# maxilevi/vits.cpp

Hardware: AMD Instinct MI355X
Metric: audio samples/sec end-to-end (ids -> fp32 PCM in HBM), vits-english architecture, batch=64 x 128 ids (higher is better)
Workload: dtype f32; 1 GPU; c3 b64x128 ref-mode f32 predicted-dur | vits-english = MMS-TTS arch, synthetic weights; batch_per_gpu=64, ids_per_utterance=128, parallelism=utterance-sharded x1

## Files before the change

### include/vits.h

```cpp
#ifndef VITS_HIP_H
#define VITS_HIP_H

#include <stddef.h>
#include <stdint.h>

#ifdef __cplusplus
#define VITS_API extern "C" __attribute__((visibility("default")))
#else
#define VITS_API __attribute__((visibility("default")))
#endif

typedef struct vits_model vits_model;

typedef struct vits_result {
    float* data;
    size_t size;
} vits_result;


VITS_API vits_model* vits_model_load_from_bytes(const char* bytes, size_t size);
VITS_API vits_model* vits_model_load_from_file(const char* path);
VITS_API void vits_free_model(vits_model* model);
VITS_API void vits_free_result(vits_result result);
VITS_API vits_result vits_model_process(vits_model* model, const char* phonemes);
// ... 204 lines not shown
    int32_t n, k[3], dilation;
    float slope;
} vits_conv_group_desc;
VITS_API int vits_op_conv_group(const vits_conv_group_desc* d, const float* x, const float* w, const float* bias, const int32_t* lens, float* y);

typedef struct vits_conv1d_desc {
    int32_t batch, cin, cout, t, t_stride;
    int32_t k, dilation, pad_left;
    int32_t pre_act;
    float pre_slope;
    int32_t post_act;
    float out_scale;
} vits_conv1d_desc;
VITS_API int vits_op_conv1d(const vits_conv1d_desc* d, const float* x, const float* w, const float* bias,
                            const float* residual, const float* accum, const int32_t* lens, float* y);

typedef struct vits_resblock_pair_desc {
    int32_t batch, channels, t, t_stride;
    int32_t k, dilation;
    float slope;
} vits_resblock_pair_desc;
VITS_API int vits_op_resblock_pair(const vits_resblock_pair_desc* d, const float* x, const float* w1, const float* b1,
                                   const float* w2, const float* b2, const int32_t* lens, float* y);

typedef struct vits_resblock_desc {
    int32_t batch, channels, t, t_stride;
    int32_t k, ndil;
    int32_t dil[3];
    float slope, out_scale;
    int32_t scale_div;
// ... 228 lines not shown
```

### vits.cpp_amd/__init__.py

```python
import ctypes as C
import json
import os

import numpy as np

_HERE = os.path.dirname(os.path.abspath(__file__))
LIB_PATH = os.environ.get("VITS_HIP_LIB", os.path.join(_HERE, "csrc", "libvits_hip.so"))

MODE_DEFAULT, MODE_REFERENCE, MODE_HF = -1, 0, 1
NOISE_REFERENCE, NOISE_COUNTER, NOISE_EXPLICIT = 0, 1, 2
SYNTH_FULL, SYNTH_TINY, SYNTH_BF16, SYNTH_SPEAKERS, SYNTH_POSTERIOR = 0, 1, 0x100, 0x200, 0x400
SYNTH_DETERMINISTIC = 0x800
DP_STOCHASTIC, DP_DETERMINISTIC = 0, 1
DP_VARIANT_PLAN, DP_VARIANT_LAT, DP_VARIANT_WIDE, DP_VARIANT_UNFUSED = 0, 1, 2, 3
RB_VARIANT_PLAN, RB_VARIANT_UNFUSED, RB_VARIANT_PAIRS, RB_VARIANT_BLOCK, RB_VARIANT_SEGMENTS = 0, 1, 2, 3, 4
FLOW_VARIANT_PLAN, FLOW_VARIANT_UNFUSED, FLOW_VARIANT_WAVENET, FLOW_VARIANT_COUPLING = 0, 1, 2, 3
UP16_VARIANT_PLAN, UP16_VARIANT_TILE, UP16_VARIANT_STREAM = 0, 1, 2
DDS_VARIANT_PLAN, DDS_VARIANT_UNFUSED, DDS_VARIANT_LAYER, DDS_VARIANT_LAT = 0, 1, 2, 3
DDS_HEAD_NONE, DDS_HEAD_FROM1, DDS_HEAD_CONV = 0, 1, 2
ATT_VARIANT_PLAN, ATT_VARIANT_VALU1024, ATT_VARIANT_VALU256, ATT_VARIANT_MFMA4, ATT_VARIANT_MFMA8, ATT_VARIANT_SHORT, ATT_VARIANT_LAT = 0, 1, 2, 3, 4, 5, 6
NC_VARIANT_PLAN, NC_VARIANT_SEPARATE, NC_VARIANT_ON_LOAD = 0, 1, 2
CONV_POST_FP32_LAYOUT, CONV_POST_STREAM = 0, 1
ARITH_F32, ARITH_BF16, ARITH_F16, ARITH_F32_SPLIT = 0, 1, 2, 3
LEVEL_NONE, LEVEL_MEASURE, LEVEL_GAIN, LEVEL_PEAK, LEVEL_LOUDNESS = 0, 1, 2, 3, 4
LIMIT_OFF, LIMIT_TRUE_PEAK = 0, 1
EDGES_OFF, EDGES_PAD, EDGES_TRIM_RELATIVE, EDGES_TRIM_ABSOLUTE = 0, 1, 2, 3
SCOPE_FLOW_VOCODER, SCOPE_ALL_CONVS = 0, 1

EXPORTED_SYMBOLS = [
    "vits_model_load_from_bytes", "vits_model_load_from_file", "vits_free_model", "vits_free_result",
    "vits_model_process", "vits_last_error", "vits_model_set_mode", "vits_model_get_mode",
    "vits_reference_noise_seed", "vits_model_process_ids", "vits_model_process_batch", "vits_free_batch_result",
    "vits_model_sync", "vits_model_tokenize", "vits_model_sampling_rate", "vits_model_vocab_size",
    "vits_model_weight_bytes", "vits_model_get_tap", "vits_synth_model_bytes", "vits_free_bytes",
    "vits_prof_enable", "vits_prof_reset", "vits_prof_report", "vits_op_conv1d", "vits_op_conv_transpose1d",
    "vits_op_rel_attention", "vits_op_add_layer_norm", "vits_device_info", "vits_set_device", "vits_model_file_reserialize",
    "vits_model_file_tokenize", "vits_pcm16_from_float", "vits_write_wav16", "vits_pcm16_from_float_device",
    "vits_model_set_arith", "vits_model_get_arith", "vits_model_file_validate", "vits_op_set_arith", "vits_op_tile_map_launches", "vits_op_set_output_fill", "vits_op_conv_group",
    "vits_model_set_arith_scope", "vits_model_get_arith_scope", "vits_model_submit_batch", "vits_model_wait", "vits_model_pending",
    "vits_model_set_ggml_tables", "vits_model_get_ggml_tables",
    "vits_model_set_speaker", "vits_model_get_speaker", "vits_model_num_speakers",
    "vits_model_speaker_embedding_size", "vits_model_get_speaker_embedding", "vits_model_add_voices", "vits_model_set_voice",
    "vits_model_clear_voices", "vits_model_num_voices",
    "vits_model_set_prosody", "vits_model_get_prosody",
    "vits_model_prepare_conversion", "vits_model_convert_batch", "vits_model_convert",
    "vits_model_align_batch", "vits_model_align", "vits_model_hop", "vits_op_align", "vits_op_resblock_pair",
    "vits_model_set_rates", "vits_model_get_rates", "vits_resample_plan", "vits_resample_taps", "vits_resample_length", "vits_op_resample",
    "vits_model_set_level", "vits_model_get_level", "vits_model_last_levels", "vits_loudness_plan", "vits_loudness_host", "vits_op_level",
    "vits_model_set_limiter", "vits_model_get_limiter", "vits_model_last_limits", "vits_limiter_plan", "vits_limiter_host", "vits_op_limit",
    "vits_model_set_edges", "vits_model_get_edges", "vits_model_last_edges", "vits_edges_plan", "vits_edges_host", "vits_op_edges",
    "vits_join_plan", "vits_join_host", "vits_op_join", "vits_split_sentences", "vits_model_process_joined", "vits_model_last_joins", "vits_model_speak",
    "vits_model_duration_predictor_kind", "vits_op_duration_predictor", "vits_op_resblock", "vits_op_resblock_plan",
    "vits_op_flow_coupling", "vits_op_flow_coupling_plan", "vits_op_upsample16", "vits_op_upsample16_plan",
# ... 45 lines not shown

class BatchResult(C.Structure):
    _fields_ = [("data", C.POINTER(C.c_float)), ("stride", C.c_size_t), ("lengths", C.POINTER(C.c_int64)),
                ("frames", C.POINTER(C.c_int64)), ("batch", C.c_size_t)]


class SpeakOpts(C.Structure):
    _fields_ = [("struct_size", C.c_uint32), ("sentence_gap_ms", C.c_float), ("paragraph_gap_ms", C.c_float), ("track_per_paragraph", C.c_int32),
                ("process", C.POINTER(ProcessOpts))]


class Conv1dDesc(C.Structure):
    _fields_ = [("batch", C.c_int32), ("cin", C.c_int32), ("cout", C.c_int32), ("t", C.c_int32), ("t_stride", C.c_int32),
                ("k", C.c_int32), ("dilation", C.c_int32), ("pad_left", C.c_int32), ("pre_act", C.c_int32),
                ("pre_slope", C.c_float), ("post_act", C.c_int32), ("out_scale", C.c_float)]


class ResblockPairDesc(C.Structure):
    _fields_ = [("batch", C.c_int32), ("channels", C.c_int32), ("t", C.c_int32), ("t_stride", C.c_int32), ("k", C.c_int32),
                ("dilation", C.c_int32), ("slope", C.c_float)]


class ConvGroupDesc(C.Structure):
    _fields_ = [("batch", C.c_int32), ("channels", C.c_int32), ("t", C.c_int32), ("t_stride", C.c_int32), ("n", C.c_int32), ("k", C.c_int32 * 3),
                ("dilation", C.c_int32), ("slope", C.c_float)]


class ResblockDesc(C.Structure):
    _fields_ = [("batch", C.c_int32), ("channels", C.c_int32), ("t", C.c_int32), ("t_stride", C.c_int32), ("k", C.c_int32), ("ndil", C.c_int32),
                ("dil", C.c_int32 * 3), ("slope", C.c_float), ("out_scale", C.c_float), ("scale_div", C.c_int32), ("variant", C.c_int32),
# ... 1059 lines not shown
              out_scale=1.0, lens=None):
    x, w = _f32(x), _f32(w)
    B, cin, T = x.shape
    cout, _, k = w.shape
    d = Conv1dDesc(B, cin, cout, T, T, k, dilation, (k - 1) * dilation // 2 if pad_left is None else pad_left,
                   0 if pre_slope is None else 1, 0.0 if pre_slope is None else pre_slope, post_act, out_scale)
    cy = cout // 2 if post_act == 2 else cout
    y = np.zeros((B, cy, T), np.float32)
    bias, residual, accum = _f32(bias), _f32(residual), _f32(accum)
    lens = None if lens is None else np.ascontiguousarray(lens, dtype=np.int32)
    if lib().vits_op_conv1d(C.byref(d), _ptr(x), _ptr(w), _ptr(bias), _ptr(residual), _ptr(accum), _ptr(lens), _ptr(y)) != 0:
        raise VitsError(last_error())
    return y


def op_resblock_pair(x, w1, b1, w2, b2, dilation, slope, lens=None):
    x, w1, w2, b1, b2 = _f32(x), _f32(w1), _f32(w2), _f32(b1), _f32(b2)
    B, ch, T = x.shape
    k = w1.shape[2]
    assert w1.shape == (ch, ch, k) and w2.shape == (ch, ch, k)
    d = ResblockPairDesc(B, ch, T, T, k, dilation, slope)
    y = np.zeros((B, ch, T), np.float32)
    lens = None if lens is None else np.ascontiguousarray(lens, dtype=np.int32)
    if lib().vits_op_resblock_pair(C.byref(d), _ptr(x), _ptr(w1), _ptr(b1), _ptr(w2), _ptr(b2), _ptr(lens), _ptr(y)) != 0:
        raise VitsError(last_error())
    return y


def _resblock_desc(B, ch, T, ts, k, dils, slope, out_scale, scale_div, variant, tiles, nr):
    dils = [int(v) for v in dils]
# ... 770 lines not shown
```

### vits.cpp_amd/csrc/abi_ops_common.h

```cpp
#pragma once
#include <algorithm>
#include <cstdint>
#include <cstring>
#include <memory>
#include <string>
#include <vector>

#include "../../include/vits.h"
#include "abi_internal.h"
#include "engine.h"

namespace vits {
extern thread_local int g_op_out_fill;
extern thread_local int g_op_arith;

inline bool refuse(const std::string& why) {
    set_err(why);
    return false;
}

struct DevMem {
    void* p = nullptr;
    DevMem() = default;
    DevMem(const DevMem&) = delete;
// ... 62 lines not shown
    for (int b = 0; b < batch; ++b)
        for (int c = 0; c < channels; ++c) {
            const T* g = &h[((size_t)b * channels + (size_t)(c / 8) * 8) * pitch + (c & 7)];
            T* d = dst + ((size_t)b * channels + c) * dst_pitch;
            for (int n = 0; n < t; ++n) d[n] = g[(size_t)n * 8];
        }
    return true;
}

struct OpKnobs {
    KernelKnobs k;
    KernelKnobsScope scope;
    OpKnobs() : k(kernel_knobs()), scope(&k) {
        k.no_tile_map = getenv("VITS_NO_TILE_MAP") != nullptr;
        k.tile_map = getenv("VITS_TILE_MAP") != nullptr;
    }
};
struct OpTileMaps {
    TileMapSet set;
    std::vector<std::unique_ptr<DevMem>> mem;
    bool add(const int32_t* len_in, const int32_t* len_out, int batch, int t_in, int t_out, int width, bool convt) {
        const KernelKnobs& kn = kernel_knobs();
        if (kn.no_tile_map || set.find(width, convt)) return true;
        std::vector<int> la(batch, t_in), lb(batch, t_out);
        if (len_in) la.assign(len_in, len_in + batch);
        if (len_out) lb.assign(len_out, len_out + batch);
        if (!kn.tile_map && !tile_map_needed(la.data(), lb.data(), batch, t_in, t_out, width, convt)) return true;
        std::vector<TileEntry> e((size_t)tile_map_count(la.data(), lb.data(), batch, width, convt) + 1);
        const int64_t n = tile_map_fill(la.data(), lb.data(), batch, width, convt, e.data());
        mem.emplace_back(new DevMem);
        if (!mem.back()->put(e.data(), e.size() * sizeof(TileEntry))) return false;
        return set.add(TileMapRef{static_cast<const TileEntry*>(mem.back()->p), (int)n, width, convt}) || refuse("too many tile widths for one length vector");
    }
    bool add_conv(const int32_t* len_in, const int32_t* len_out, int batch, int t_in, int t_out, bool convt) {
        return add(len_in, len_out, batch, t_in, t_out, tile_shape(TILE_128x128).bn(), convt) && add(len_in, len_out, batch, t_in, t_out, tile_shape(TILE_64x256).bn(), convt);
    }
};

struct Conv {
    PackedConv pc;
    DevMem w, wl, w16, b;
};
inline bool upload_conv(Conv& c, const float* w, const float* bias, size_t bias_n, int cout, int cin, int taps, int epi, int ct_stride, int arith, bool l16_always = false) {
    PackedConv& pc = c.pc;
    const ConvPackDims pd = conv_pack_dims(cout, cin, taps, epi, ct_stride);
    pc.cin = cin, pc.cout = cout, pc.kt = pd.kt, pc.epi = epi, pc.ct_stride = ct_stride;
    pc.rows = pd.rows, pc.mtiles_used = pd.mtiles_used, pc.mtiles = pd.mtiles, pc.nchunks = pd.nchunks;
    if (bias) {
        if (!c.b.put(bias, bias_n * 4)) return false;
        pc.bias = c.b.f();
// ... 34 lines not shown
```

### vits.cpp_amd/csrc/abi_ops_conv.cpp

```cpp
#include <cstdio>

#include "abi_ops_common.h"

namespace vits {
thread_local int g_op_arith = VITS_ARITH_F32;
thread_local int g_op_out_fill = 0;
}
using namespace vits;

namespace {
bool split3_nan(DevMem& d, int batch, int channels, int ts, Split3Ref* r) {
    if (!d.fill((size_t)batch * 3 * channels * ts * 2, 0xFF)) return false;
    r->p = d.h();
    r->ts = ts;
    r->ps = (int64_t)channels * ts;
    r->bs = 3 * r->ps;
    return true;
}
std::string split_refusal(int cin, int cout, int k, int dil) {
    char m[200] = "";
    if (cin < 128 || (cin & 31)) std::snprintf(m, sizeof(m), "VITS_ARITH_F32_SPLIT: c_in = %d is not taken by the split kernels (a multiple of 32, at least 128)", cin);
    else if (cout < 128 || (cout & 127)) std::snprintf(m, sizeof(m), "VITS_ARITH_F32_SPLIT: c_out = %d is not taken by the split kernels (a multiple of 128)", cout);
    else if (k != 3 && k != 7 && k != 11) std::snprintf(m, sizeof(m), "VITS_ARITH_F32_SPLIT: k = %d taps are not taken by the split kernels (3, 7 or 11)", k);
    else if (dil != 1 && dil != 3 && dil != 5) std::snprintf(m, sizeof(m), "VITS_ARITH_F32_SPLIT: dilation %d is not taken by the split kernels (1, 3 or 5)", dil);
// ... 97 lines not shown
        c.len_in = c.len_out = dl.i();
        c.maps = &maps.set;
        c.batch = B;
        c.t_in = c.t_out = d->t;
        c.dil = d->dilation;
        c.pad_l = (k * d->dilation - d->dilation) / 2;
        c.pre_act = 1, c.slope = d->slope, c.post_act = 2, c.post_slope = d->slope;
        pw[i] = &cv[i].pc;
    }
    return finish(launch_conv_group(pw, cc, n, nullptr), "vits_op_conv_group") && dy.get(y, per * n * 4) ? 0 : -1;
    VITS_CATCH(-1)
}

VITS_API uint64_t vits_op_tile_map_launches(void) { return tile_map_launches().load(std::memory_order_relaxed); }

VITS_API int vits_op_conv1d(const vits_conv1d_desc* d, const float* x, const float* w, const float* bias, const float* residual, const float* accum,
                            const int32_t* lens, float* y) {
    VITS_TRY
    if (!d || !x || !w || !y) return fail("null argument");
    const int arith = g_op_arith;
    if (arith == VITS_ARITH_F32_SPLIT) return op_conv1d_split(d, x, w, bias, residual, accum, lens, y);
    OpKnobs op_knobs;
    OpTileMaps maps;
    const int gate = d->post_act == 2;
    const int cy = gate ? d->cout / 2 : d->cout;
    Conv cv;
    DevMem dx, dy, dr, da, dl, x16;
    const size_t nx = (size_t)d->batch * d->cin * d->t_stride * 4, ny = (size_t)d->batch * cy * d->t_stride * 4;
    if (!upload_conv(cv, w, bias, d->cout, d->cout, d->cin, d->k, gate ? EPI_GATE : EPI_STD, 0, arith)) return -1;
    if (!dx.put(x, nx) || !dy.fill(ny, g_op_out_fill) || !dl.put_opt(lens, (size_t)d->batch * 4)) return -1;
    if ((residual && !dr.put(residual, ny)) || (accum && !da.put(accum, ny))) return -1;
    if (arith != VITS_ARITH_F32 && !x16.fill(group16_bytes(d->batch, d->cin, d->t), 0)) return -1;
    ConvCall c;
    c.x = tref(dx.f(), d->cin, d->t_stride);
    c.y = tref(dy.f(), cy, d->t_stride);
    if (residual) c.res = tref(dr.f(), cy, d->t_stride);
    if (accum) c.acc = tref(da.f(), cy, d->t_stride);
    c.len_in = dl.i();
    c.len_out = dl.i();
    c.batch = d->batch;
    c.t_in = c.t_out = d->t;
    c.dil = d->dilation;
    c.pad_l = d->pad_left;
    c.pre_act = d->pre_act;
    c.slope = d->pre_slope;
    c.post_act = d->post_act == 1 ? 1 : 0;
    c.scale = d->out_scale;
    if (arith == VITS_ARITH_F32) {
        if (!maps.add_conv(lens, lens, d->batch, d->t, d->t, false)) return -1;
        c.maps = &maps.set;
    }
    return finish(conv_transparent(cv.pc, c, arith, x16)) && dy.get(y, ny) ? 0 : -1;
    VITS_CATCH(-1)
}

VITS_API int vits_op_resblock_pair(const vits_resblock_pair_desc* d, const float* x, const float* w1, const float* b1, const float* w2, const float* b2,
                                   const int32_t* lens, float* y) {
    VITS_TRY
    if (!d || !x || !w1 || !w2 || !y) return fail("null argument");
    if (g_op_arith != VITS_ARITH_F32 && g_op_arith != VITS_ARITH_F32_SPLIT) return fail("vits_op_resblock_pair: VITS_ARITH_F32 or VITS_ARITH_F32_SPLIT only");
    if (!shape_lens_ok(lens, d->batch, d->t, d->t_stride)) return fail("vits_op_resblock_pair: 0 <= lens[b] <= t <= t_stride is required");
    if (d->channels < 1 || d->k < 1 || !(d->k & 1) || d->dilation < 1) return fail("vits_op_resblock_pair: an odd tap count and a dilation >= 1 are required");
    const int C = d->channels, k = d->k;
    const size_t n = (size_t)d->batch * C * d->t_stride * 4;
    DevMem dx, dy, dl;
    if (!dx.put(x, n) || !dy.fill(n, g_op_out_fill) || !dl.put_opt(lens, (size_t)d->batch * 4)) return -1;
    const TensorRef bx = tref(dx.f(), C, d->t_stride), by = tref(dy.f(), C, d->t_stride);
// ... 441 lines not shown
```

### vits.cpp_amd/csrc/conv_mfma.hip

```cpp
#include <hip/hip_runtime.h>
#include <type_traits>

#include <algorithm>
#include <atomic>
#include <cmath>
#include <cstdint>
#include <cstdlib>
#include <cstring>

#include "kernel_common.h"
#include "kernels.h"

#ifndef VITS_CONV_PART
#define VITS_CONV_PART 0
#endif

namespace vits {


constexpr int CK = 32;

struct ConvParams {
    const float* x;
    int64_t x_bs;
// ... 1127 lines not shown
    const size_t lds = pl.lds;
#define VITS_TILE_ARM(LABEL, T)                                                      \
    LABEL:                                                                           \
        if constexpr (conv_tile_exists(EPI, KT, DIL, DB, T)) {                       \
            constexpr TileShape ts = tile_shape(T);                                  \
            return launch_lds<&conv_mfma_kernel<KT, DIL, DB, ts.wm, ts.wn, ts.mr, ts.nr, EPI>>(grid, dim3(DB ? 320 : 256), lds, s, p); \
        } else {                                                                     \
            return hipErrorInvalidValue;                                             \
        }
    switch (pl.tile) {
        VITS_TILE_ARM(case TILE_128x128, TILE_128x128)
        VITS_TILE_ARM(case TILE_64x256, TILE_64x256)
        VITS_TILE_ARM(case TILE_32x256, TILE_32x256)
        VITS_TILE_ARM(case TILE_64x64, TILE_64x64)
        VITS_TILE_ARM(case TILE_NARROW, TILE_NARROW)
        VITS_TILE_ARM(default, TILE_32x64)
    }
#undef VITS_TILE_ARM
}

#define VITS_GO(K, D, E)                                                                      \
    do {                                                                                      \
        if (w.kt == K && pl.dil_ct == D) {                                                    \
            if ((D) != 0 && pl.db) return launch_tile<K, D, (D) != 0, E>(pl, p, s);           \
            return launch_tile<K, D, false, E>(pl, p, s);                                     \
        }                                                                                     \
    } while (0)
#define VITS_LAUNCHER(K) hipError_t launch_conv_k##K(const PackedConv& w, const ConvPlan& pl, const ConvParams& p, hipStream_t s)
#define VITS_LAUNCHER_BODY(K) \
    VITS_LAUNCHER(K) { VITS_GO(K, 1, EPI_STD); VITS_GO(K, 3, EPI_STD); VITS_GO(K, 5, EPI_STD); VITS_GO(K, 0, EPI_STD); return hipErrorInvalidValue; }
// ... 111 lines not shown
    p.ln_gamma = c.ln_gamma;
    p.ln_beta = c.ln_beta;
    p.ln_eps = c.ln_eps;
    p.ln_out = c.ln_out.p;
    p.lo_bs = c.ln_out.bs;
    p.lo_cs = c.ln_out.cs;
    p.dil = pl.dil;
    p.pad_l = w.epi == EPI_CONVT ? 0 : c.pad_l;
    p.lds_off = pl.lds_off;
    p.xw = pl.xw;
    p.nbuf = pl.nbuf;
    p.oneshot = pl.oneshot;
}

hipError_t launch_conv(const PackedConv& w, const ConvCall& c, hipStream_t s) {
    const ConvPlan pl = plan_conv(w, c);
    if (!pl.ok) return hipErrorInvalidValue;
    ConvParams p;
    make_conv_params(w, c, pl, p);
    if (c.ln_gamma && (!c.ln_beta || !c.ln_out.p || !pl.ln_ok)) return hipErrorInvalidValue;
    if (pl.tile == TILE_LAT16) return launch_lat16(w, pl, p, s);
    if (p.tmap && p.tmap_n == 0) return hipSuccess;
#ifdef VITS_MICRO_KT
    if ((VITS_MICRO_DIL) != 0 && pl.db) return launch_tile<VITS_MICRO_KT, VITS_MICRO_DIL, (VITS_MICRO_DIL) != 0, EPI_STD>(pl, p, s);
    return launch_tile<VITS_MICRO_KT, VITS_MICRO_DIL, false, EPI_STD>(pl, p, s);
#else
    if (w.epi == EPI_CONVT) {
        VITS_GO(2, -1, EPI_CONVT);
    } else if (w.epi == EPI_GATE) {
        VITS_GO(5, 1, EPI_GATE);
        VITS_GO(5, 0, EPI_GATE);
// ... 21 lines not shown
```

### vits.cpp_amd/csrc/conv_plan.cpp

```cpp
#include "conv_plan.h"

namespace vits {

static int resolve_conv_tile(const PackedConv& w, const ConvCall& c) {
    const KernelKnobs& kn = kernel_knobs();
    const int ncols_max = conv_ncols(w, c);
    if (c.tile >= 0) return c.tile;
    const bool small_t = ncols_max <= 128 || (kn.narrow_tiles && w.rows <= kn.narrow_tiles);
    int tile = small_t ? TILE_32x64 : TILE_32x256;
    if (w.epi == EPI_GATE || w.rows % 64 == 0) tile = small_t ? TILE_64x64 : TILE_64x256;
    if (w.epi != EPI_GATE && w.rows % 128 == 0 && kn.tile128) tile = TILE_128x128;
    auto blocks = [&](int tl) { return tile_blocks(tile_shape(tl), ncols_max, w.mtiles_used, c.batch); };
    if (w.epi == EPI_GATE) {
        if (blocks(tile) < kSmallGridBlocks) tile = TILE_64x64;
    } else {
        const int64_t min_blocks = kn.min_blocks > 0 ? kn.min_blocks : (w.kt <= 3 ? 2 * kSmallGridBlocks : kSmallGridBlocks);
        if (blocks(tile) < min_blocks && (tile == TILE_128x128 || tile == TILE_64x256)) tile = TILE_64x64;
        if (blocks(tile) < min_blocks && (tile == TILE_64x64 || tile == TILE_32x256)) tile = TILE_32x64;
    }
    if (w.epi != EPI_CONVT) {
        const int dil_eff = conv_dil(w, c);
        const bool shape_ok = dil_eff == 1 && conv_narrow_shape(w.epi, w.kt);
        const int64_t nb = blocks(tile);
        const bool k1_short = kn.narrow_k1 > 0 && w.epi == EPI_STD && w.kt == 1 && ncols_max <= kn.narrow_k1;
// ... 46 lines not shown
    p.ln_ok = !p.ln_why;
    if (p.tile == TILE_LAT16) {
        p.ok = p.ok && p.pitch && w.wp_l16;
        p.xw = p.pitch;
        p.gx = (ncols_max + 15) / 16, p.gy = (w.mtiles_used + 1) / 2, p.block = 256;
        p.lds = lat_bytes + (c.ln_gamma ? ln_bytes : 0);
    } else {
        p.ok = p.ok && aspan <= 64 && p.dil_ct != kNoKernel && conv_tile_exists(w.epi, w.kt, p.dil_ct, p.db, p.tile);
        p.gx = (ncols_max + ts.bn() - 1) / ts.bn(), p.gy = (w.mtiles_used + ts.bm() - 1) / ts.bm(), p.block = p.db ? 320 : 256;
        p.lds = p.db ? p.nbuf * row_bytes : (size_t)kConvCK * p.xw * sizeof(float);
    }
    p.gz = c.batch;
    return p;
}

bool conv_ln_on_load_ok(const PackedConv& w, const ConvCall& c) { return plan_conv(w, c).ln_ok; }

bool conv_lat16_candidate(int epi, int kt, int cin) {
    return (epi == EPI_STD || (epi == EPI_GATE && kt == 5)) && (int64_t)kt * cin >= 64;
}

bool conv_group_supported(const PackedConv& w, int dil) {
    return w.epi == EPI_STD && (w.kt == 11 || w.kt == 7 || w.kt == 3) && (dil == 1 || dil == 3 || dil == 5) && w.rows % 128 == 0 && w.cin % kConvCK == 0;
}

bool conv_split_candidate(int epi, int kt, int cin, int cout) {
    return epi == EPI_STD && (kt == 3 || kt == 7 || kt == 11) && cin >= 128 && (cin & 31) == 0 && (cout & 127) == 0;
}
bool conv_split_supported(const PackedConv& w, int dil) {
    return w.wps && conv_split_candidate(w.epi, w.kt, w.cin, w.cout) && (dil == 1 || dil == 3 || dil == 5);
// ... 93 lines not shown
```

### vits.cpp_amd/csrc/conv_plan.h

```cpp
#pragma once
#include "kernels.h"

namespace vits {

constexpr int kConvCK = 32;
constexpr int kNoKernel = -99;
#ifndef VITS_XWP_GRAN
#define VITS_XWP_GRAN 16
#endif
template <class Call>
inline int conv_ncols(const PackedConv& w, const Call& c) { return w.epi == EPI_CONVT ? c.t_in + 1 : c.t_out; }
template <class Call>
inline int conv_dil(const PackedConv& w, const Call& c) { return w.epi == EPI_CONVT ? -1 : (w.kt == 1 ? 1 : c.dil); }
struct TileShape {
    int wm, wn, mr, nr;
    constexpr int bn() const { return wn * nr * 32; }
    constexpr int bm() const { return wm * mr; }
};
constexpr TileShape tile_shape(int tile) {
    switch (tile) {
        case TILE_128x128: return {2, 2, 2, 2};
        case TILE_64x256: return {1, 4, 2, 2};
        case TILE_32x256: return {1, 4, 1, 2};
        case TILE_64x64: return {1, 4, 2, 1};
        case TILE_LAT16:
        case TILE_NARROW: return {4, 1, 1, 1};
        default: return {1, 4, 1, 1};
    }
}
constexpr TileShape tile16_shape(int tile) {
    switch (tile) {
        case 0: return {2, 2, 2, 4};
        case 1: return {1, 4, 2, 2};
        case 2: return {1, 4, 1, 2};
        case 3: return {1, 4, 2, 1};
        case 5: return {2, 2, 2, 2};
        case 6: return {4, 1, 1, 4};
        default: return {1, 4, 1, 1};
    }
}
constexpr bool conv_tile_mapped(int tile) { return tile != TILE_LAT16 && tile != TILE_NARROW && tile_shape(tile).mr * tile_shape(tile).nr >= 4; }
// ... 24 lines not shown
    if (epi == EPI_CONVT) return kt == 2 ? -1 : kNoKernel;
    if (epi == EPI_GATE) return kt != 5 ? kNoKernel : dil == 1 ? 1 : 0;
    if (kt == 1) return 1;
    if (kt == 5) return dil == 1 ? 1 : 0;
    if (kt == 3 || kt == 7 || kt == 11) return dil == 1 || dil == 3 || dil == 5 ? dil : 0;
    return kNoKernel;
#endif
}
constexpr bool conv_narrow_shape(int epi, int kt) { return (epi == EPI_STD && kt <= 3) || (epi == EPI_GATE && kt == 5); }
constexpr bool conv_tile_exists(int epi, int kt, int dil_ct, bool db, int tile) {
    switch (tile) {
        case TILE_64x256:
        case TILE_64x64: return true;
        case TILE_NARROW: return db && dil_ct == 1 && conv_narrow_shape(epi, kt);
        case TILE_LAT16: return false;
        default: return epi != EPI_GATE;
    }
}
constexpr bool conv_lat16_exists(int epi, int pitch) { return pitch && (epi == EPI_STD || (epi == EPI_GATE && pitch == 24)); }
enum Conv16Epi : int { C16_STD = 0, C16_GATE = 1, C16_CONVT = 2, C16_GROUP = 3, C16_CONVT_GROUP = 4 };
constexpr int conv16_template_dil(int epi16, int kt, int dil) {
    const bool rb = kt == 3 || kt == 7 || kt == 11;
    if (epi16 == C16_CONVT || epi16 == C16_CONVT_GROUP) return kt == 2 ? -1 : kNoKernel;
    if (epi16 == C16_GATE) return kt == 5 || kt == 3 ? 0 : kNoKernel;
    if (kt == 1) return 1;
    if (epi16 == C16_STD) return rb || kt == 5 ? 0 : kNoKernel;
    return rb ? (dil == 1 || dil == 3 || dil == 5 ? dil : 0) : kt == 5 ? 0 : kNoKernel;
}
constexpr bool conv16_tile_exists(int epi16, int dil_ct, int tile) {
    const bool group = epi16 == C16_GROUP || epi16 == C16_CONVT_GROUP;
// ... 11 lines not shown

struct ConvPlan {
    bool ok = false;
    int tile = 0;
    int dil = 1;
    int dil_ct = 0;
    bool db = false;
    int gx = 0, gy = 0, gz = 0, block = 0;
    size_t lds = 0;
    int xw = 0, lds_off = 0, nbuf = 2, oneshot = 0;
    int pitch = 0;
    bool ln_ok = false;
    const char* ln_why = nullptr;
};
ConvPlan plan_conv(const PackedConv& w, const ConvCall& c, int forced_tile = -1);
struct Conv16LatPlan {
    int wm = 0, nr = 0, pitch = 0, gx = 0, gy = 0, gz = 0, block = 0;
    size_t lds = 0;
};
Conv16LatPlan plan_conv16_lat(int cin, int cout, int kt, int dil, int shape, int tmax, int nz);
Conv16LatPlan plan_conv16_lat_group(int dil, int tmax, int batch);
struct Conv16Plan {
    bool ok = false;
    bool lat = false;
    int epi16 = 0, chosen = 0, tile = 0;
    int part = 0;
    int dil = 1, dil_ct = 0, gx = 0, gy = 0, gz = 0;
    size_t lds = 0;
    int xwp = 0, lds_off = 0, nbuf = 2;
    Conv16LatPlan l;
// ... 5 lines not shown
```

### vits.cpp_amd/csrc/engine.cpp

```cpp
#include <cmath>
#include <numeric>

#include "engine_internal.h"

namespace vits {

hipError_t Engine::conv16(const char* name, const PackedConv& w, const Conv16Call& c, hipStream_t stream, double bytes) {
    if (prof.on) {
        const Conv16Plan pl = plan_conv16(w, c);
        const bool group = c.yg || c.y16.p;
        char full[160];
        std::snprintf(full, sizeof(full), "%s|k%d|d%d|T%d|e%d%s|c%dx%d", name, w.kt, pl.dil, pl.tile, w.epi, group ? "g" : "", w.cin,
                      w.cout);
        const int64_t tot_in = c.sum_in >= 0 ? c.sum_in : (int64_t)c.batch * c.t_in;
        const int64_t tot_out = c.sum_out >= 0 ? c.sum_out : (int64_t)c.batch * c.t_out;
        const int64_t cols = w.epi == EPI_CONVT ? tot_in : tot_out;
        prof.begin(full, 2.0 * (double)w.rows * (double)w.cin * (double)w.kt * (double)cols, bytes, stream, true);
    }
    hipError_t e = launch_conv16(w, c, arith_now_, stream);
    prof.end(stream);
    return e;
}

hipError_t Engine::conv16_transparent(const char* name, const PackedConv& w, const ConvCall& c, hipStream_t stream) {
// ... 41 lines not shown
    hipStream_t stream = on ? on : this->stream;
    if (c.xs3.p) {
        if (prof.on) {
            char full[160];
            std::snprintf(full, sizeof(full), "%s|k%d|d%d|S128|e0|c%dx%d", name, w.kt, c.dil, w.cin, w.cout);
            const int64_t tot = c.sum_out >= 0 ? c.sum_out : (int64_t)c.batch * c.t_out;
            const double bytes = (double)tot * (6.0 * w.cin + (double)w.cout * (4.0 * ((c.y.p ? 1 : 0) + (c.res.p ? 1 : 0) + (c.acc.p ? 1 : 0)) + (c.ys3.p ? 6.0 : 0.0))) + (double)w.bytes_s;
            prof.begin(full, conv_flops(w, c, tot), bytes, stream, true);
        }
        hipError_t e = launch_conv_split(w, c, stream);
        prof.end(stream);
        return e;
    }
    if (arith_now_ != VITS_ARITH_F32 && w.wp16) return conv16_transparent(name, w, c, stream);
    if (prof.on) {
        const ConvPlan pl = plan_conv(w, c);
        char full[160];
        std::snprintf(full, sizeof(full), "%s|k%d|d%d|t%d|e%d|c%dx%d", name, w.kt, pl.dil, pl.tile, w.epi, w.cin,
                      w.cout);
        const int64_t tot_in = c.sum_in >= 0 ? c.sum_in : (int64_t)c.batch * c.t_in;
        const int64_t tot_out = c.sum_out >= 0 ? c.sum_out : (int64_t)c.batch * c.t_out;
        const int64_t cols = w.epi == EPI_CONVT ? tot_in : tot_out;
        const int cout_stored = w.epi == EPI_GATE ? w.cout / 2 : w.cout;
        double bytes = 4.0 * ((double)w.cin * tot_in + (double)cout_stored * tot_out * (1 + (c.res.p ? 1 : 0) + (c.acc.p ? 1 : 0) + (c.y2 ? 1 : 0))) + (double)w.bytes;
        prof.begin(full, conv_flops(w, c, cols), bytes, stream, true);
    }
    hipError_t e = launch_conv(w, c, stream);
    prof.end(stream);
    return e;
}

// ... 739 lines not shown
            if (!kn.tile_map && dense_blocks < kSmallGridBlocks) return;
            const int vo = convt ? vec + 1 : vec;
            for (int b = 0; b < B; ++b) la[b] = c.win_len(wi, vec, b), lb[b] = c.win_len(wi, vo, b);
            if (!kn.tile_map && !tile_map_needed(la.data(), lb.data(), B, smax(vec), smax(vo), width, convt)) return;
            const int64_t n = tile_map_count(la.data(), lb.data(), B, width, convt);
            c.tm_jobs.push_back({(int)wi, vec, width, convt, c.tm_total, n});
            c.tm_total += n;
        };
        auto conv_width = [&](const PackedConv& w, int vec, int dil) {
            const bool convt = w.epi == EPI_CONVT;
            ConvCall shape;
            shape.batch = B;
            shape.t_in = smax(vec);
            shape.t_out = smax(convt ? vec + 1 : vec);
            shape.dil = dil;
            const ConvPlan pl = plan_conv(w, shape);
            if (!pl.ok || !conv_tile_mapped(pl.tile)) return;
            want(vec, tile_shape(pl.tile).bn(), convt, (int64_t)pl.gx * pl.gy * pl.gz);
        };
        conv_width(dec_pre_, 0, 1);
        for (int i = 0; i < n_up; ++i) {
            const UpStageW& U = ups_[i];
            const int C = U.channels, vec = i + 1;
            conv_width(U.up, i, 1);
            for (size_t j = 0; j < nk; ++j) {
                const ResBlockW& R = U.rbs[j];
                const int kind = j < 3 ? rb32_kind(R, C) : 0;
                const bool fused = kind >= 1;
                if (kind == 2) {
                    const RbBlock32Plan pl = plan_rbblock32(C, R.k, B, smax(vec));
                    want(vec, rbblock32_geom(C, pl.nr).bo, false, (int64_t)pl.gx * pl.gy);
// ... 491 lines not shown
```

### vits.cpp_amd/csrc/kernels.h

```cpp
#pragma once
#include <hip/hip_runtime.h>
#include <hip/hip_ext.h>

#include <algorithm>
#include <atomic>
#include <cstdint>
#include <cstdlib>
#include <string>
#include <vector>

#include "tile_map.h"

struct vits_edges_desc;

namespace vits {

struct KernelKnobs {
    int narrow_tiles = 64;
    int tile128 = 1;
    int min_blocks = 0;
    bool no_narrow = false;
    int narrow_k1 = 1 << 30;
    int nbuf = 0;
    bool no_oneshot = false;
// ... 29 lines not shown
    bool no_dds_lat = false;
    int dds_lat_max_blocks = 96;
    bool no_dp_det_fuse = false;
    int dp_det_lat_max_blocks = 96;
    int lat16h_group_shape = 21;
    bool no_lat16h_group = false;
    bool no_lat16h_pre = false;
    bool no_lat16h = false;
    int lat16h_max_tiles = 2048;
    int lat16h_max_tiles_c128 = 0;
    int lat16h_shape = 21;
    bool no_lat16 = false;
    int lat16_max_waves = 768;
    bool no_tile_map = false;
    bool tile_map = false;
    static KernelKnobs from_env() {
        KernelKnobs k;
        auto num = [](const char* name, int& v) {
            if (const char* e = getenv(name)) v = atoi(e);
        };
        auto flag = [](const char* name, bool& v) { v = getenv(name) != nullptr; };
        num("VITS_NARROW_TILES", k.narrow_tiles);
        flag("VITS_NO_DDS_LAT", k.no_dds_lat);
        flag("VITS_NO_LN_FUSE", k.no_ln_fuse);
        flag("VITS_NO_RB_SUM3", k.no_rb_sum3);
        flag("VITS_RB_SUM3_BLOCK_ONLY", k.rb_sum3_block_only);
        flag("VITS_RB_SUM3_IN_ORDER", k.rb_sum3_in_order);
        flag("VITS_NO_RB_SUM3_F32", k.no_rb_sum3_f32);
        flag("VITS_NO_RBB_GROUP3", k.no_rbb_group3);
        flag("VITS_NO_RBB_GROUP3_C64", k.no_rbb_group3_c64);
// ... 27 lines not shown
        num("VITS_FLOW_NARROW_MAX", k.flow_narrow_max);
        num("VITS_RB16_NARROW_MAX", k.rb16_narrow_max);
        num("VITS_CONVT16_SPLIT_MAX", k.convt16_split_max);
        num("VITS_CONVT16_R128", k.convt16_r128);
        flag("VITS_NO_LAT16", k.no_lat16);
        flag("VITS_NO_LAT16H", k.no_lat16h);
        flag("VITS_NO_LAT16H_PRE", k.no_lat16h_pre);
        flag("VITS_NO_LAT16H_GROUP", k.no_lat16h_group);
        num("VITS_LAT16H_GROUP_SHAPE", k.lat16h_group_shape);
        num("VITS_LAT16H_MAX_TILES", k.lat16h_max_tiles);
        num("VITS_LAT16H_MAX_TILES_C128", k.lat16h_max_tiles_c128);
        num("VITS_LAT16H_SHAPE", k.lat16h_shape);
        num("VITS_LAT16_MAX_WAVES", k.lat16_max_waves);
        flag("VITS_NO_TILE_MAP", k.no_tile_map);
        flag("VITS_TILE_MAP", k.tile_map);
        return k;
    }
};
namespace detail {
inline thread_local const KernelKnobs* tl_kernel_knobs = nullptr;
}
inline const KernelKnobs& kernel_knobs() {
    if (detail::tl_kernel_knobs) return *detail::tl_kernel_knobs;
    static const KernelKnobs process_default = KernelKnobs::from_env();
    return process_default;
}
struct KernelKnobsScope {
    const KernelKnobs* prev;
    explicit KernelKnobsScope(const KernelKnobs* k) : prev(detail::tl_kernel_knobs) { detail::tl_kernel_knobs = k; }
    ~KernelKnobsScope() { detail::tl_kernel_knobs = prev; }
// ... 60 lines not shown

struct TensorRef {
    float* p = nullptr;
    int64_t bs = 0;
    int32_t cs = 0;
};

enum ConvEpilogue : int { EPI_STD = 0, EPI_GATE = 1, EPI_CONVT = 2 };
enum ConvTile : int {
    TILE_128x128 = 0,
    TILE_64x256 = 1,
    TILE_32x256 = 2,
    TILE_64x64 = 3,
    TILE_32x64 = 4,
    TILE_NARROW = 5,
    TILE_LAT16 = 6
};

struct PackedConv {
    float* wp = nullptr;
    float* bias = nullptr;
    int64_t bias_rs = 0;
    int cin = 0, cout = 0, kt = 0;
    int rows = 0;
    int mtiles = 0;
    int mtiles_used = 0;
    int nchunks = 0;
    int epi = EPI_STD;
    int ct_stride = 0;
    int64_t bytes = 0;
    uint16_t* wp16 = nullptr;
// ... 503 lines not shown
```

Baseline: 51.48 million samples/s.

## Add tall 256x64 MFMA conv tile for wide fp32 standard convolutions

Adds a TILE_TALL conv tile, 256 output rows by 64 columns with a 320-thread block, and a planner that picks it for exact-fp32 standard convs with c_out a multiple of 256, c_in of at least 128, aligned operands, a large enough grid and supported tap/dilation combinations. All launch and tile-map paths now go through plan_conv_launch, so qualifying convs use the new tile by default. The taller tile is meant to reuse each input tile across more output channels and cut input re-reads. In exchange it needs more LDS per block and may lower occupancy. Also adds op-level entry points for a leaky post-activation, a second output and a plan query, used for testing.

Measured after the change: 51.80 million samples/s (median of 6 runs). About the same (+0.6%).

```diff
diff --git a/include/vits.h b/include/vits.h
--- a/include/vits.h
+++ b/include/vits.h
@@ -242,6 +242,14 @@
 } vits_conv1d_desc;
 VITS_API int vits_op_conv1d(const vits_conv1d_desc* d, const float* x, const float* w, const float* bias,
                             const float* residual, const float* accum, const int32_t* lens, float* y);
+VITS_API int vits_op_conv1d_act(const vits_conv1d_desc* d, int32_t post_leaky, float post_slope, const float* x, const float* w, const float* bias,
+                                const float* residual, const float* accum, const int32_t* lens, float* y, float* y2);
+typedef struct vits_conv1d_plan {
+    int32_t ok, tile, tile_rows, tile_cols;
+    int32_t grid_x, grid_y, grid_z, block;
+    int64_t lds;
+} vits_conv1d_plan;
+VITS_API int vits_op_conv1d_plan(const vits_conv1d_desc* d, vits_conv1d_plan* out);
 
 typedef struct vits_resblock_pair_desc {
     int32_t batch, channels, t, t_stride;
diff --git a/vits.cpp_amd/__init__.py b/vits.cpp_amd/__init__.py
--- a/vits.cpp_amd/__init__.py
+++ b/vits.cpp_amd/__init__.py
@@ -37,6 +37,7 @@
     "vits_op_rel_attention", "vits_op_add_layer_norm", "vits_device_info", "vits_set_device", "vits_model_file_reserialize",
     "vits_model_file_tokenize", "vits_pcm16_from_float", "vits_write_wav16", "vits_pcm16_from_float_device",
     "vits_model_set_arith", "vits_model_get_arith", "vits_model_file_validate", "vits_op_set_arith", "vits_op_tile_map_launches", "vits_op_set_output_fill", "vits_op_conv_group",
+    "vits_op_conv1d_act", "vits_op_conv1d_plan",
     "vits_model_set_arith_scope", "vits_model_get_arith_scope", "vits_model_submit_batch", "vits_model_wait", "vits_model_pending",
     "vits_model_set_ggml_tables", "vits_model_get_ggml_tables",
     "vits_model_set_speaker", "vits_model_get_speaker", "vits_model_num_speakers",
@@ -112,6 +113,11 @@
     _fields_ = [("batch", C.c_int32), ("cin", C.c_int32), ("cout", C.c_int32), ("t", C.c_int32), ("t_stride", C.c_int32),
                 ("k", C.c_int32), ("dilation", C.c_int32), ("pad_left", C.c_int32), ("pre_act", C.c_int32),
                 ("pre_slope", C.c_float), ("post_act", C.c_int32), ("out_scale", C.c_float)]
+
+
+class Conv1dPlan(C.Structure):
+    _fields_ = [("ok", C.c_int32), ("tile", C.c_int32), ("tile_rows", C.c_int32), ("tile_cols", C.c_int32), ("grid_x", C.c_int32), ("grid_y", C.c_int32),
+                ("grid_z", C.c_int32), ("block", C.c_int32), ("lds", C.c_int64)]
 
 
 class ResblockPairDesc(C.Structure):
@@ -1201,6 +1207,34 @@
     return y
 
 
+def op_conv1d_act(x, w, bias=None, dilation=1, pre_slope=None, post_leaky=False, post_slope=0.0, want_y2=False, residual=None, accum=None, out_scale=1.0, lens=None):
+    x, w = _f32(x), _f32(w)
+    B, cin, T = x.shape
+    cout, _, k = w.shape
+    d = Conv1dDesc(B, cin, cout, T, T, k, dilation, (k - 1) * dilation // 2, 0 if pre_slope is None else 1, 0.0 if pre_slope is None else pre_slope, 0, out_scale)
+    y = np.zeros((B, cout, T), np.float32)
+    y2 = np.zeros((B, cout, T), np.float32) if want_y2 else None
+    bias, residual, accum = _f32(bias), _f32(residual), _f32(accum)
+    lens = None if lens is None else np.ascontiguousarray(lens, dtype=np.int32)
+    f = lib().vits_op_conv1d_act
+    f.restype, f.argtypes = C.c_int32, [C.POINTER(Conv1dDesc), C.c_int32, C.c_float] + [C.c_void_p] * 8
+    if f(C.byref(d), int(bool(post_leaky)), post_slope, _ptr(x), _ptr(w), _ptr(bias), _ptr(residual), _ptr(accum), _ptr(lens), _ptr(y), _ptr(y2)) != 0:
+        raise VitsError(last_error())
+    return (y, y2) if want_y2 else y
+
+
+def op_conv1d_plan(cin, cout, k, t, batch=1, dilation=1):
+    d = Conv1dDesc(batch, cin, cout, t, t, k, dilation, (k - 1) * dilation // 2, 0, 0.0, 0, 1.0)
+    p = Conv1dPlan()
+    f = lib().vits_op_conv1d_plan
+    f.restype, f.argtypes = C.c_int32, [C.POINTER(Conv1dDesc), C.POINTER(Conv1dPlan)]
+    if f(C.byref(d), C.byref(p)) != 0:
+        raise VitsError(last_error())
+    out = {n: getattr(p, n) for n in ("ok", "tile", "tile_rows", "tile_cols", "block", "lds")}
+    out["grid"] = (p.grid_x, p.grid_y, p.grid_z)
+    return out
+
+
 def op_resblock_pair(x, w1, b1, w2, b2, dilation, slope, lens=None):
     x, w1, w2, b1, b2 = _f32(x), _f32(w1), _f32(w2), _f32(b1), _f32(b2)
     B, ch, T = x.shape
diff --git a/vits.cpp_amd/csrc/abi_ops_common.h b/vits.cpp_amd/csrc/abi_ops_common.h
--- a/vits.cpp_amd/csrc/abi_ops_common.h
+++ b/vits.cpp_amd/csrc/abi_ops_common.h
@@ -100,6 +100,8 @@
     OpKnobs() : k(kernel_knobs()), scope(&k) {
         k.no_tile_map = getenv("VITS_NO_TILE_MAP") != nullptr;
         k.tile_map = getenv("VITS_TILE_MAP") != nullptr;
+        k.no_tall_tile = getenv("VITS_NO_TALL_TILE") != nullptr;
+        k.tall_tile = getenv("VITS_TALL_TILE") != nullptr;
     }
 };
 struct OpTileMaps {
@@ -119,7 +121,8 @@
         return set.add(TileMapRef{static_cast<const TileEntry*>(mem.back()->p), (int)n, width, convt}) || refuse("too many tile widths for one length vector");
     }
     bool add_conv(const int32_t* len_in, const int32_t* len_out, int batch, int t_in, int t_out, bool convt) {
-        return add(len_in, len_out, batch, t_in, t_out, tile_shape(TILE_128x128).bn(), convt) && add(len_in, len_out, batch, t_in, t_out, tile_shape(TILE_64x256).bn(), convt);
+        return add(len_in, len_out, batch, t_in, t_out, tile_shape(TILE_128x128).bn(), convt) && add(len_in, len_out, batch, t_in, t_out, tile_shape(TILE_64x256).bn(), convt) &&
+               (convt || add(len_in, len_out, batch, t_in, t_out, tile_shape(TILE_TALL).bn(), false));
     }
 };
 
diff --git a/vits.cpp_amd/csrc/abi_ops_conv.cpp b/vits.cpp_amd/csrc/abi_ops_conv.cpp
--- a/vits.cpp_amd/csrc/abi_ops_conv.cpp
+++ b/vits.cpp_amd/csrc/abi_ops_conv.cpp
@@ -135,21 +135,23 @@
 
 VITS_API uint64_t vits_op_tile_map_launches(void) { return tile_map_launches().load(std::memory_order_relaxed); }
 
-VITS_API int vits_op_conv1d(const vits_conv1d_desc* d, const float* x, const float* w, const float* bias, const float* residual, const float* accum,
-                            const int32_t* lens, float* y) {
+static int op_conv1d_run(const vits_conv1d_desc* d, int post_leaky, float post_slope, const float* x, const float* w, const float* bias, const float* residual, const float* accum,
+                         const int32_t* lens, float* y, float* y2) {
     VITS_TRY
     if (!d || !x || !w || !y) return fail("null argument");
     const int arith = g_op_arith;
+    if ((post_leaky || y2) && (arith != VITS_ARITH_F32 || d->post_act != 0)) return fail("vits_op_conv1d_act: post_leaky / y2 are the fp32 standard conv's (post_act 0, VITS_ARITH_F32)");
     if (arith == VITS_ARITH_F32_SPLIT) return op_conv1d_split(d, x, w, bias, residual, accum, lens, y);
     OpKnobs op_knobs;
     OpTileMaps maps;
     const int gate = d->post_act == 2;
     const int cy = gate ? d->cout / 2 : d->cout;
     Conv cv;
-    DevMem dx, dy, dr, da, dl, x16;
+    DevMem dx, dy, dy2, dr, da, dl, x16;
     const size_t nx = (size_t)d->batch * d->cin * d->t_stride * 4, ny = (size_t)d->batch * cy * d->t_stride * 4;
     if (!upload_conv(cv, w, bias, d->cout, d->cout, d->cin, d->k, gate ? EPI_GATE : EPI_STD, 0, arith)) return -1;
     if (!dx.put(x, nx) || !dy.fill(ny, g_op_out_fill) || !dl.put_opt(lens, (size_t)d->batch * 4)) return -1;
+    if (y2 && !dy2.fill(ny, g_op_out_fill)) return -1;
     if ((residual && !dr.put(residual, ny)) || (accum && !da.put(accum, ny))) return -1;
     if (arith != VITS_ARITH_F32 && !x16.fill(group16_bytes(d->batch, d->cin, d->t), 0)) return -1;
     ConvCall c;
@@ -165,13 +167,43 @@
     c.pad_l = d->pad_left;
     c.pre_act = d->pre_act;
     c.slope = d->pre_slope;
-    c.post_act = d->post_act == 1 ? 1 : 0;
+    c.post_act = post_leaky ? 2 : d->post_act == 1 ? 1 : 0;
+    c.post_slope = post_slope;
+    if (y2) c.y2 = dy2.f();
     c.scale = d->out_scale;
     if (arith == VITS_ARITH_F32) {
         if (!maps.add_conv(lens, lens, d->batch, d->t, d->t, false)) return -1;
         c.maps = &maps.set;
     }
-    return finish(conv_transparent(cv.pc, c, arith, x16)) && dy.get(y, ny) ? 0 : -1;
+    return finish(conv_transparent(cv.pc, c, arith, x16)) && dy.get(y, ny) && (!y2 || dy2.get(y2, ny)) ? 0 : -1;
+    VITS_CATCH(-1)
+}
+
+VITS_API int vits_op_conv1d(const vits_conv1d_desc* d, const float* x, const float* w, const float* bias, const float* residual, const float* accum,
+                            const int32_t* lens, float* y) {
+    return op_conv1d_run(d, 0, 0.f, x, w, bias, residual, accum, lens, y, nullptr);
+}
+
+VITS_API int vits_op_conv1d_act(const vits_conv1d_desc* d, int32_t post_leaky, float post_slope, const float* x, const float* w, const float* bias, const float* residual,
+                                const float* accum, const int32_t* lens, float* y, float* y2) {
+    return op_conv1d_run(d, post_leaky, post_slope, x, w, bias, residual, accum, lens, y, y2);
+}
+
+VITS_API int vits_op_conv1d_plan(const vits_conv1d_desc* d, vits_conv1d_plan* out) {
+    VITS_TRY
+    if (!d || !out) return fail("null argument");
+    OpKnobs op_knobs;
+    const int gate = d->post_act == 2;
+    const ConvPackDims pd = conv_pack_dims(d->cout, d->cin, d->k, gate ? EPI_GATE : EPI_STD, 0);
+    PackedConv pc;
+    pc.cin = d->cin, pc.cout = d->cout, pc.kt = pd.kt, pc.epi = gate ? EPI_GATE : EPI_STD;
+    pc.rows = pd.rows, pc.mtiles_used = pd.mtiles_used, pc.mtiles = pd.mtiles, pc.nchunks = pd.nchunks;
+    ConvCall c;
+    c.batch = d->batch, c.t_in = c.t_out = d->t, c.dil = d->dilation, c.pad_l = d->pad_left;
+    const ConvPlan pl = plan_conv_launch(pc, c, g_op_arith);
+    out->ok = pl.ok, out->tile = pl.tile, out->tile_rows = 32 * tile_shape(pl.tile).bm(), out->tile_cols = tile_shape(pl.tile).bn();
+    out->grid_x = pl.gx, out->grid_y = pl.gy, out->grid_z = pl.gz, out->block = pl.block, out->lds = (int64_t)pl.lds;
+    return 0;
     VITS_CATCH(-1)
 }
 
diff --git a/vits.cpp_amd/csrc/conv_mfma.hip b/vits.cpp_amd/csrc/conv_mfma.hip
--- a/vits.cpp_amd/csrc/conv_mfma.hip
+++ b/vits.cpp_amd/csrc/conv_mfma.hip
@@ -1165,6 +1165,7 @@
         VITS_TILE_ARM(case TILE_32x256, TILE_32x256)
         VITS_TILE_ARM(case TILE_64x64, TILE_64x64)
         VITS_TILE_ARM(case TILE_NARROW, TILE_NARROW)
+        VITS_TILE_ARM(case TILE_TALL, TILE_TALL)
         VITS_TILE_ARM(default, TILE_32x64)
     }
 #undef VITS_TILE_ARM
@@ -1306,7 +1307,7 @@
 }
 
 hipError_t launch_conv(const PackedConv& w, const ConvCall& c, hipStream_t s) {
-    const ConvPlan pl = plan_conv(w, c);
+    const ConvPlan pl = plan_conv_launch(w, c);
     if (!pl.ok) return hipErrorInvalidValue;
     ConvParams p;
     make_conv_params(w, c, pl, p);
diff --git a/vits.cpp_amd/csrc/conv_plan.cpp b/vits.cpp_amd/csrc/conv_plan.cpp
--- a/vits.cpp_amd/csrc/conv_plan.cpp
+++ b/vits.cpp_amd/csrc/conv_plan.cpp
@@ -84,6 +84,47 @@
     return p;
 }
 
+ConvTallPlan plan_conv_tall(const PackedConv& w, const ConvCall& c, int arith) {
+    const KernelKnobs& kn = kernel_knobs();
+    ConvTallPlan p;
+    p.tile = TILE_TALL;
+    const TileShape ts = tile_shape(TILE_TALL);
+    const int ncols_max = conv_ncols(w, c);
+    p.dil = conv_dil(w, c);
+    p.dil_ct = conv_template_dil(w.epi, w.kt, p.dil);
+    p.db = p.dil_ct != 0 && p.dil_ct != kNoKernel && w.nchunks >= kn.db_min;
+    const int span = (w.kt - 1) * (p.dil < 0 ? -p.dil : p.dil);
+    p.xw = ts.bn() + span;
+    p.lds_off = 0;
+    const size_t row_bytes = (size_t)kConvCK * padded_xw(p.xw) * sizeof(float);
+    p.nbuf = kn.nbuf == 2 || kn.nbuf == 3 ? kn.nbuf : 2;
+    if (w.nchunks < 2 || p.nbuf * row_bytes > 150 * 1024) p.nbuf = 2;
+    p.gx = (ncols_max + ts.bn() - 1) / ts.bn(), p.gy = (w.mtiles_used + ts.bm() - 1) / ts.bm(), p.gz = c.batch, p.block = 320;
+    p.lds = p.nbuf * row_bytes;
+    p.pitch = lat16_pitch(span);
+    p.ln_why = "the 256 x 64 tile has no LayerNorm on load";
+    auto al16 = [](const TensorRef& t) { return (reinterpret_cast<uintptr_t>(t.p) & 15) == 0 && (t.cs & 3) == 0 && (t.bs & 3) == 0; };
+    p.why = kn.no_tall_tile                                              ? "VITS_NO_TALL_TILE"
+            : arith != 0 || c.xs3.p || c.ys3.p                           ? "not the exact-fp32 arithmetic"
+            : w.epi != EPI_STD                                           ? "not a standard conv (epilogue)"
+            : c.ln_gamma                                                 ? "LayerNorm on load"
+            : c.tile >= 0                                                ? "the call names its tile"
+            : !p.db || !conv_tile_exists(w.epi, w.kt, p.dil_ct, p.db, TILE_TALL) ? "no producer-wave kernel at a compile-time dilation for these taps"
+            : w.rows % 256 != 0 || w.mtiles_used * 32 != w.rows          ? "c_out is not a multiple of 256"
+            : w.cin < 128 || w.cin % kConvCK != 0                        ? "c_in < 128 or not whole chunks"
+            : !al16(c.x) || !al16(c.y) || !al16(c.res) || !al16(c.acc) || (reinterpret_cast<uintptr_t>(c.y2) & 15) != 0 ? "operands not 16-byte aligned"
+            : !kn.tall_tile && tile_blocks(ts, ncols_max, w.mtiles_used, c.batch) < kSmallGridBlocks ? "a small grid"
+            : p.lds > 150 * 1024                                         ? "the input tile passes 150 KB of LDS"
+                                                                         : nullptr;
+    p.ok = !p.why;
+    return p;
+}
+
+ConvPlan plan_conv_launch(const PackedConv& w, const ConvCall& c, int arith) {
+    const ConvTallPlan t = plan_conv_tall(w, c, arith);
+    return t.ok ? static_cast<const ConvPlan&>(t) : plan_conv(w, c);
+}
+
 bool conv_ln_on_load_ok(const PackedConv& w, const ConvCall& c) { return plan_conv(w, c).ln_ok; }
 
 bool conv_lat16_candidate(int epi, int kt, int cin) {
diff --git a/vits.cpp_amd/csrc/conv_plan.h b/vits.cpp_amd/csrc/conv_plan.h
--- a/vits.cpp_amd/csrc/conv_plan.h
+++ b/vits.cpp_amd/csrc/conv_plan.h
@@ -25,6 +25,7 @@
         case TILE_64x64: return {1, 4, 2, 1};
         case TILE_LAT16:
         case TILE_NARROW: return {4, 1, 1, 1};
+        case TILE_TALL: return {4, 1, 2, 2};
         default: return {1, 4, 1, 1};
     }
 }
@@ -79,6 +80,7 @@
         case TILE_64x64: return true;
         case TILE_NARROW: return db && dil_ct == 1 && conv_narrow_shape(epi, kt);
         case TILE_LAT16: return false;
+        case TILE_TALL: return epi == EPI_STD && db && (kt == 3 || kt == 7 || kt == 11) && (dil_ct == 1 || dil_ct == 3 || dil_ct == 5);
         default: return epi != EPI_GATE;
     }
 }
@@ -120,6 +122,11 @@
     const char* ln_why = nullptr;
 };
 ConvPlan plan_conv(const PackedConv& w, const ConvCall& c, int forced_tile = -1);
+struct ConvTallPlan : ConvPlan {
+    const char* why = nullptr;
+};
+ConvTallPlan plan_conv_tall(const PackedConv& w, const ConvCall& c, int arith = 0);
+ConvPlan plan_conv_launch(const PackedConv& w, const ConvCall& c, int arith = 0);
 struct Conv16LatPlan {
     int wm = 0, nr = 0, pitch = 0, gx = 0, gy = 0, gz = 0, block = 0;
     size_t lds = 0;
diff --git a/vits.cpp_amd/csrc/engine.cpp b/vits.cpp_amd/csrc/engine.cpp
--- a/vits.cpp_amd/csrc/engine.cpp
+++ b/vits.cpp_amd/csrc/engine.cpp
@@ -79,7 +79,7 @@
     }
     if (arith_now_ != VITS_ARITH_F32 && w.wp16) return conv16_transparent(name, w, c, stream);
     if (prof.on) {
-        const ConvPlan pl = plan_conv(w, c);
+        const ConvPlan pl = plan_conv_launch(w, c);
         char full[160];
         std::snprintf(full, sizeof(full), "%s|k%d|d%d|t%d|e%d|c%dx%d", name, w.kt, pl.dil, pl.tile, w.epi, w.cin,
                       w.cout);
@@ -849,7 +849,7 @@
             shape.t_in = smax(vec);
             shape.t_out = smax(convt ? vec + 1 : vec);
             shape.dil = dil;
-            const ConvPlan pl = plan_conv(w, shape);
+            const ConvPlan pl = plan_conv_launch(w, shape);
             if (!pl.ok || !conv_tile_mapped(pl.tile)) return;
             want(vec, tile_shape(pl.tile).bn(), convt, (int64_t)pl.gx * pl.gy * pl.gz);
         };
diff --git a/vits.cpp_amd/csrc/kernels.h b/vits.cpp_amd/csrc/kernels.h
--- a/vits.cpp_amd/csrc/kernels.h
+++ b/vits.cpp_amd/csrc/kernels.h
@@ -67,6 +67,8 @@
     int lat16_max_waves = 768;
     bool no_tile_map = false;
     bool tile_map = false;
+    bool no_tall_tile = false;
+    bool tall_tile = false;
     static KernelKnobs from_env() {
         KernelKnobs k;
         auto num = [](const char* name, int& v) {
@@ -124,6 +126,8 @@
         num("VITS_LAT16_MAX_WAVES", k.lat16_max_waves);
         flag("VITS_NO_TILE_MAP", k.no_tile_map);
         flag("VITS_TILE_MAP", k.tile_map);
+        flag("VITS_NO_TALL_TILE", k.no_tall_tile);
+        flag("VITS_TALL_TILE", k.tall_tile);
         return k;
     }
 };
@@ -214,7 +218,8 @@
     TILE_64x64 = 3,
     TILE_32x64 = 4,
     TILE_NARROW = 5,
-    TILE_LAT16 = 6
+    TILE_LAT16 = 6,
+    TILE_TALL = 7
 };
 
 struct PackedConv {
```
